# HugoZHL/MEVI

Measured on AMD Instinct MI355X. Metric: queries/sec @ MRR@10-match, MSMARCO dev, 1/2/4/8 MI355X, higher is better.
Workload: dtype f16+f32; 1 GPU; C2 dense arm (faiss_search.py Flat): 6980 x 768 f32 queries x 8841823 x 768 f32 docs, exact inner-product top-1000; queries=6980, docs=8841823, dim=768, topk=1000, parallelism=single GPU

## Files before the change

include/mevi_hip.h:

```cpp
#ifndef MEVI_HIP_H
#define MEVI_HIP_H

#include <stddef.h>
#include <stdint.h>

#ifdef __cplusplus
extern "C" {
#endif

#define MEVI_OK 0
#define MEVI_ERR_INVALID_ARG (-1)
#define MEVI_ERR_UNSUPPORTED (-2)
#define MEVI_ERR_WORKSPACE (-3)
#define MEVI_ERR_HIP (-4)

int mevi_abi_version(void);

const char *mevi_last_error(void);

size_t mevi_ip_topk_workspace_bytes(int64_t nq, int64_t dim, int64_t k);

int mevi_ip_topk_f32(const float *q, int64_t nq, const float *docs, int64_t nd,
                     int64_t dim, int64_t k, int64_t id_offset,
                     float *out_score, int64_t *out_id, void *workspace,
// ... 259 lines not shown
                            int64_t R, int pq, int32_t *labels, float *proba, void *workspace, size_t workspace_bytes,
                            void *stream);

size_t mevi_cluster_means_workspace_bytes(int64_t n, int64_t dim, int64_t K);
int mevi_cluster_means_f32(const float *x, int64_t n, int64_t dim, const int32_t *codes, int64_t code_stride,
                           int64_t K, const float *old_centroids, float *centroids, int32_t *counts, double *sum_sq,
                           void *workspace, size_t workspace_bytes, void *stream);

typedef struct mevi_ip_topk_stats {
  int64_t n_chunks;
  int64_t n_failed_queries;
  int64_t n_fallback_chunks;
  double filter_ms;
  double compact_ms;
  double filter_flops;
  double max_err_ratio;
  double err_bound;
  int64_t n_second_pass_queries;
  int64_t n_filter_candidates;
  int64_t max_launch_candidates;
  int64_t n_list_overflows;
  int64_t n_i8_queries;
  int64_t n_i8_unproven;
} mevi_ip_topk_stats;
int64_t mevi_ip_filter_tile_walk(int64_t n_dpairs, int64_t n_qtiles, int label, int32_t *dpair, int32_t *qtile);
void mevi_ip_topk_set_growth(double growth);
void mevi_ip_topk_set_profiling(int enable);
void mevi_ip_topk_get_stats(mevi_ip_topk_stats *out);

int64_t mevi_format_f32_list(const float *v, int64_t n, char *out, int64_t cap);
int64_t mevi_format_i64_list(const int64_t *v, int64_t n, char *out, int64_t cap);
int mevi_format_ranked_rows(const int64_t *ids, const float *scores, int64_t rows, int64_t k, char *out, int64_t row_cap,
                            int64_t *lens, int32_t threads);
int64_t mevi_parse_i64_list(const char *s, int64_t len, int64_t *out, int64_t cap);
int64_t mevi_parse_f64_list(const char *s, int64_t len, double *out, int64_t cap);

int64_t mevi_parse_tsv_columns(const char *buf, int64_t len, int32_t col_q, int32_t col_i, int32_t col_f, int64_t *q_span,
                               int64_t *seg_i, int64_t *vals_i, int64_t cap_i, int64_t *seg_f, double *vals_f,
                               int64_t cap_f, int64_t cap_lines);

int mevi_cluster_ranks_i32(const int32_t *codes, int64_t n_docs, int64_t M, const int64_t *docs, const int64_t *seg,
                           int64_t nq, const int32_t *beam, int64_t R, int32_t n_clusters, int32_t *out_ranks,
                           uint64_t *first_bad, void *stream);
int mevi_ensemble_rank_f64(const int64_t *seg_dense, const int64_t *docs_dense, const double *scores_dense,
                           const int32_t *cranks_dense, const int64_t *fine_row, const int64_t *seg_fine,
                           const int64_t *docs_fine, const double *scores_fine, int64_t nq, int64_t max_entries,
                           int32_t n_clusters, const double *term, double punish, const int64_t *out_seg,
                           int64_t *out_docs, int32_t *out_n, int32_t *err, void *stream);
// ... 8 lines not shown
```

mevi_amd/csrc/ip_topk.hip:

```cpp

#include "mfma_pp_f16x16.h"

#include <float.h>
#include <math.h>
#include <string.h>
#include <vector>

namespace mevi {
namespace {

constexpr int MAX_SORT = 16384;

struct TopkGeom {
  int k;
  int S;
  int cap;
};

static inline int next_pow2(int x) {
  int p = 1;
  while (p < x) p <<= 1;
  return p;
}

// ... 546 lines not shown
        base += __popcll(mask);
      }
    }
  for (int i = base + lane; i < k; i += 64) row[i] = (i == k - 1) ? T : 0ull;
  if (lane == 0) {
    tau[q] = (T != 0ull) ? key_score(T) : -INFINITY;
    count[q] = 0u;
    if (c_raw > (unsigned int)cap) failed[q] = 1u;
  }
}

template <int KPL>
__global__ __launch_bounds__(256) void rank_tau_kernel(const unsigned long long *__restrict__ buf, int nq, int S, int k, int rank,
                                                      float *__restrict__ tau, float *__restrict__ tau_s) {
  const int lane = threadIdx.x & 63;
  const int q = blockIdx.x * 4 + (int)(threadIdx.x >> 6);
  if (q >= nq) return;
  const unsigned long long *row = buf + (size_t)q * S;
  unsigned long long key[KPL];
#pragma unroll
  for (int j = 0; j < KPL; ++j) key[j] = (64 * j + lane < k) ? row[64 * j + lane] : 0ull;
  const int nj = (k + 63) >> 6;
  unsigned long long T = 0ull;
  for (int b = 63; b >= 0; --b) {
    const unsigned long long cand = T | (1ull << b);
    int cnt = 0;
#pragma unroll
    for (int jb = 0; jb < KPL / 8; ++jb)
      if (8 * jb < nj) {
#pragma unroll
        for (int jj = 0; jj < 8; ++jj) cnt += __popcll(__ballot(key[8 * jb + jj] >= cand));
      }
    if (cnt >= rank) T = cand;
  }
  if (lane == 0) {
    const float t = (T != 0ull) ? key_score(T) : -INFINITY;
    tau_s[q] = t;
    if (tau) tau[q] = t;
  }
}

__global__ __launch_bounds__(256) void sample_check_kernel(const float *__restrict__ tau, const float *__restrict__ tau_s,
                                                          unsigned int *__restrict__ failed, int nq) {
  const int q = blockIdx.x * 256 + threadIdx.x;
  if (q < nq && !(tau[q] > tau_s[q]) && tau_s[q] > -INFINITY) failed[q] = 1u;
}

__global__ __launch_bounds__(256) void sort_lists_kernel(unsigned long long *__restrict__ buf, int S, int k) {
  extern __shared__ __attribute__((aligned(16))) unsigned long long skeys[];
  const int t = threadIdx.x;
  unsigned long long *row = buf + (size_t)blockIdx.x * S;
  int P = 64;
  while (P < k) P <<= 1;
  for (int i = t; i < P; i += 256) skeys[i] = (i < k) ? row[i] : 0ull;
  __syncthreads();
  bitonic_sort_desc<256>(skeys, P, t);
// ... 942 lines not shown
    if (!ok) failed[q] = 1u;
  }
}

__global__ __launch_bounds__(256) void count_candidates_kernel(const unsigned int *__restrict__ count, int nq, int cap,
                                                              unsigned long long *__restrict__ out) {
  const int q = blockIdx.x * 256 + threadIdx.x;
  const unsigned int c = q < nq ? count[q] : 0u;
  unsigned long long sum = c;
  unsigned int mx = c, over = c > (unsigned int)cap ? 1u : 0u;
#pragma unroll
  for (int off = 32; off > 0; off >>= 1) {
    sum += ((unsigned long long)(unsigned int)__shfl_xor((int)(sum >> 32), off) << 32) | (unsigned int)__shfl_xor((int)sum, off);
    mx = max(mx, (unsigned int)__shfl_xor((int)mx, off));
    over += (unsigned int)__shfl_xor((int)over, off);
  }
  if ((threadIdx.x & 63) == 0 && sum != 0ull) {
    atomicAdd(out, sum);
    atomicMax(out + 1, (unsigned long long)mx);
    if (over) atomicAdd(out + 2, (unsigned long long)over);
  }
}

class Carver {
  char *base_;
  size_t used_ = 0;
 public:
  explicit Carver(void *base) : base_(static_cast<char *>(base)) {}
  template <typename T> T *take(size_t count) {
    T *p = base_ ? reinterpret_cast<T *>(base_ + used_) : nullptr;
    used_ += align_up(count * sizeof(T), 256);
    return p;
  }
  size_t used() const { return used_; }
};
template <typename F> static size_t carved_bytes(F &&carve) {
  Carver count(nullptr);
  carve(count);
  return count.used();
}

struct SearchState {
  unsigned long long *buf;
  unsigned int *count;
  float *tau;
  unsigned int *failed;
// ... 10 lines not shown
  SearchState st, fb;
  float *qsub; int *fidx;
  char *spare;
};
static ExactWs carve_exact(Carver &c, int64_t nq, int64_t dim, const TopkGeom &g) {
  return {carve_state(c, nq, g), carve_state(c, nq, g), c.take<float>((size_t)nq * dim), c.take<int>(nq), c.take<char>(256)};
}

struct QuerySide {
  float *image;
  float *norm, *inv, *delta, *n16;
  double *shift;
  unsigned int *err_bits;
};
static QuerySide carve_query_side(Carver &c, int64_t nq, size_t image_bytes) {
  QuerySide s = {reinterpret_cast<float *>(c.take<char>(image_bytes)), c.take<float>(nq + 1), c.take<float>(nq + 1),
                 c.take<float>(nq + 1), c.take<float>(nq + 1), c.take<double>(nq), nullptr};
  if (s.norm) s.err_bits = reinterpret_cast<unsigned int *>(s.norm + nq);
  return s;
}

thread_local double g_growth = 0.0;
thread_local int g_profile = 0;
thread_local mevi_ip_topk_stats g_stats = {0, 0, 0, 0.0, 0.0, 0.0, 0.0, 0.0, 0, 0, 0, 0};
thread_local std::vector<hipEvent_t> g_events;
thread_local std::vector<long long> g_chunk_rows;

static void profile_mark(hipStream_t stream) {
  if (!g_profile) return;
  hipEvent_t e;
  if (hipEventCreate(&e) != hipSuccess) return;
  (void)hipEventRecord(e, stream);
  g_events.push_back(e);
}

static void profile_collect() {
  for (size_t i = 0; i + 3 <= g_events.size(); i += 3) {
    float f = 0.f, c = 0.f;
    (void)hipEventElapsedTime(&f, g_events[i], g_events[i + 1]);
    (void)hipEventElapsedTime(&c, g_events[i + 1], g_events[i + 2]);
    g_stats.filter_ms += f;
    g_stats.compact_ms += c;
    if (getenv("MEVI_IP_TOPK_TRACE") && i / 3 < g_chunk_rows.size())
      fprintf(stderr, "ip_topk launch %zu: %lld rows  filter %.3f ms  compact %.3f ms\n", i / 3, g_chunk_rows[i / 3], f, c);
  }
  g_chunk_rows.clear();
  for (hipEvent_t e : g_events) (void)hipEventDestroy(e);
  g_events.clear();
}

enum class PassKind { ExactF32, F16Image, I8Image };
struct PassArgs {
  PassKind kind;
  const float *Q; int64_t nq;
  const float *D; int64_t nd; int dim;
  TopkGeom g; uint32_t id_base; SearchState st;
  bool guaranteed;
  unsigned long long *cand = nullptr;
  const float *row_scale = nullptr, *qub = nullptr;
};

enum class FilterGrid { PerTile, PerCU, SmallStream };
struct FilterChoice {
  const void *fn;
  size_t lds;
  int qt, ni16;
  FilterGrid grid;
};

static bool choose_filter(PassKind kind, int64_t nq, int dim, FilterChoice &f) {
  const bool h1 = kind != PassKind::ExactF32;
  const int ni = 2;
  static const bool shape32_f = [] { const char *e = getenv("MEVI_IP_FILTER_MFMA"); return e && atoi(e) == 32; }();
  static const int qt_pin = [] { const char *e = getenv("MEVI_IP_FILTER_QT"); return e ? atoi(e) : 0; }();
  const bool k16shape = h1 && !shape32_f && dim % 64 == 0;
  int ni16 = 8;
  if (k16shape) {
    ni16 = nq <= 64 ? 2 : (nq <= 128 ? 4 : 8);
    if (qt_pin == 256 || qt_pin == 128 || qt_pin == 64) ni16 = qt_pin / 32;
    const int nunits = dim / 32;
    if (ni16 == 2 && nunits < 5) ni16 = 4;
    if (ni16 == 4 && nunits < 4) ni16 = 8;
  }
// ... 25 lines not shown
}

static int64_t run_pass(const PassArgs &a, hipStream_t stream) {
  const int64_t nq = a.nq, nd = a.nd;
  const TopkGeom &g = a.g;
  const SearchState &st = a.st;
  const bool guaranteed = a.guaranteed;
  const long long total = nq * (long long)g.k;
  const long long init_n = total > nq ? total : nq;
  const int n_tickets = TICKET_SLOTS * 8;
  hipLaunchKernelGGL(init_state_kernel, dim3((unsigned)(((init_n > n_tickets ? init_n : n_tickets) + 255) / 256)), dim3(256), 0, stream,
                     st.buf, st.count, st.tau, st.failed, (long long)nq, g.S, g.k, st.tickets, n_tickets);
  const size_t compact_lds = (size_t)g.S * 8 + 2048;
  if (compact_lds > 65536) {
    if (hipFuncSetAttribute(reinterpret_cast<const void *>(compact_kernel),
                            hipFuncAttributeMaxDynamicSharedMemorySize, (int)compact_lds) != hipSuccess) {
      set_error("ip_topk: cannot raise dynamic LDS to %zu bytes", compact_lds);
      return -1;
    }
  }
  FilterChoice f;
  if (!choose_filter(a.kind, nq, a.dim, f)) return -1;
  const int n_qtiles = (int)((nq + f.qt - 1) / f.qt);
  double growth_div = 3.0;
  if (const char *e = getenv("MEVI_IP_TOPK_GROWTH_DIV")) {
    const double v = atof(e);
    if (v >= 1.05 && v <= 64.0) growth_div = v;
  }
  double growth = g_growth > 0.0 ? g_growth : (double)g.cap / (growth_div * g.k);
  if (growth < 1.0) growth = 1.0;
  if (g_growth <= 0.0 && !getenv("MEVI_IP_TOPK_GROWTH_DIV") && !guaranteed) {
    const double keys = (double)nq * (double)g.k * 60e-9 * 1e3, t_launch = 0.2;
    double best = growth, best_cost = (keys * growth + t_launch) / log(1.0 + growth);
    for (double cand = 1.0; cand < growth; cand += 0.25) {
      const double c = (keys * cand + t_launch) / log(1.0 + cand);
      if (c < best_cost * 0.99) best = cand, best_cost = c;
    }
    growth = best;
  }
  int64_t cap_docs = (g.cap / (2 * BM)) * (2 * BM);
  if (const char *e = getenv("MEVI_IP_TOPK_FIRST_CHUNK")) {
    const int64_t v = atoll(e) / (2 * BM) * (2 * BM);
    if (v >= 2 * BM && v < cap_docs) cap_docs = v;
  }
  if (hipFuncSetAttribute(f.fn, hipFuncAttributeMaxDynamicSharedMemorySize, (int)f.lds) != hipSuccess) {
    set_error("ip_topk: cannot raise dynamic LDS to %zu bytes", f.lds);
    return -1;
  }
  int n_cu = 256;
  {
    int dev = 0, v = 0;
    if (hipGetDevice(&dev) == hipSuccess &&
        hipDeviceGetAttribute(&v, hipDeviceAttributeMultiprocessorCount, dev) == hipSuccess && v >= 8)
      n_cu = v;
  }
  static const int cu_cap = [] { const char *e = getenv("MEVI_IP_FILTER_CUS"); return e ? atoi(e) : 0; }();
  if (cu_cap >= 8 && cu_cap < n_cu) n_cu = cu_cap / 8 * 8;
  static const int sample_mode = [] { const char *e = getenv("MEVI_IP_SAMPLE_TAU"); return e ? atoi(e) : -1; }();
  const bool sample_on = sample_mode == 1 || (sample_mode != 0 && nq <= 1024);
  double s_c = 0.0;
  int64_t n_sample = 0;
  bool sampled = false;
  if (sample_on && !guaranteed && g.k <= 4096 && g.k >= 32) {
    const double r = g.k / 2 < 16 ? 16.0 : (g.k / 2 > 96 ? 96.0 : (double)(g.k / 2));
    double c = r >= 96.0 ? 3.0 : 8.0;
    const double c_fit = (double)g.cap / ((double)g.k * (1.0 + 8.0 / sqrt(r)));
    if (c_fit < c) c = c_fit;
    if (c >= 1.5 && (1.0 - 1.0 / c) * sqrt(r) >= 4.5) {
      s_c = c;
      n_sample = (int64_t)ceil(r * (double)nd / (c * (double)g.k));
    }
  }
  int64_t seen = 0, launches = 0;
  while (seen < nd) {
    int64_t chunk = cap_docs;
    if (!guaranteed && seen >= g.k) {
      int64_t grown = (int64_t)((double)seen * growth);
      grown = grown / (2 * BM) * (2 * BM);
      if (grown > chunk) chunk = grown;
    }
    if (chunk > nd - seen) chunk = nd - seen;
    double expect_per_q = seen >= g.k ? (double)g.k * (double)chunk / (double)seen : (double)chunk;
    if (s_c > 0.0 && !sampled && seen >= n_sample && seen >= g.k && chunk < nd - seen) {
      const int64_t rank = (int64_t)ceil(s_c * (double)g.k * (double)seen / (double)nd);
      if (rank >= 16 && rank <= g.k) {
        hipLaunchKernelGGL(rank_tau_kernel<64>, dim3((unsigned)((nq + 3) / 4)), dim3(256), 0, stream, st.buf, (int)nq, g.S, g.k, (int)rank,
                           st.tau, st.tau_s);
        sampled = true;
        chunk = nd - seen;
        expect_per_q = s_c * (double)g.k;
      }
    }
    const int64_t n_dtiles = (chunk + 2 * BM - 1) / (2 * BM);
    const int64_t nwg = n_dtiles * n_qtiles;
    if (nwg > 0x7fffffffLL) {
      set_error("ip_topk: grid too large (%lld workgroups)", (long long)nwg);
      return -1;
    }
    profile_mark(stream);
    {
      int nq_i = (int)nq, n_dp = (int)n_dtiles, n_qt = n_qtiles;
      long long d0 = (long long)seen, d1 = (long long)(seen + chunk);
      const float *tau_c = st.tau;
      void *args[18] = {(void *)&a.Q, &nq_i, (void *)&a.D, &d0, &d1, (void *)&a.dim, (void *)&tau_c, (void *)&st.buf,
                        (void *)&st.count, (void *)&g.S, (void *)&g.k, (void *)&g.cap, (void *)&a.id_base};
      unsigned grid = (unsigned)nwg;
      int flush_mask = H16_FLUSH_EVERY - 1;
      unsigned int *tickets = st.tickets + 8 * (launches & 1), *tickets_next = st.tickets + 8 * ((launches + 1) & 1);
      if (f.grid == FilterGrid::SmallStream) {
        const int64_t nb = (chunk + 255) / 256;
        grid = (unsigned)(nb < n_cu ? nb : n_cu);
        args[13] = (void *)&a.row_scale;
        args[14] = (void *)&a.qub;
      } else {
// ... 2 lines not shown
          grid = (unsigned)(8 * per_xcd);
        }
        args[13] = &n_qt;
        args[14] = &n_dp;
      }
      if (f.ni16) {
        const double per_q = expect_per_q;
        const double r = per_q / (double)chunk * 64.0 * 16.0 * (double)f.ni16;
        int T = H16_FLUSH_EVERY;
        while (T > 1 && T * r > 56.0) T >>= 1;
        flush_mask = T - 1;
        args[15] = &flush_mask;
        args[16] = (void *)&tickets;
        args[17] = (void *)&tickets_next;
      }
      if (hipLaunchKernel(f.fn, dim3(grid), dim3(PP_THREADS), args, f.lds, stream) != hipSuccess) {
        set_error("ip_topk: filter kernel launch failed");
        return -1;
      }
    }
    profile_mark(stream);
    if (a.cand)
      hipLaunchKernelGGL(count_candidates_kernel, dim3((unsigned)((nq + 255) / 256)), dim3(256), 0, stream, st.count, (int)nq, g.cap, a.cand);
    {
      const int nq_i = (int)nq;
      static const bool wave_compact = [] { const char *e = getenv("MEVI_IP_TOPK_COMPACT"); return !(e && strcmp(e, "lds") == 0); }();
      if (wave_compact)
        hipLaunchKernelGGL(compact_wave_kernel<64>, dim3((unsigned)((nq + 3) / 4)), dim3(256), 0, stream, st.buf, st.count, st.tau,
                           st.failed, nq_i, g.S, g.k, g.cap);
      hipLaunchKernelGGL(compact_kernel, dim3((unsigned)(nq < 8 * n_cu ? nq : 8 * n_cu)), dim3(256), compact_lds, stream,
                         st.buf, st.count, st.tau, st.failed, nq_i, g.S, g.k, g.cap);
    }
    if (sampled && seen + chunk >= nd)
      hipLaunchKernelGGL(sample_check_kernel, dim3((unsigned)((nq + 255) / 256)), dim3(256), 0, stream, st.tau, st.tau_s, st.failed, (int)nq);
    profile_mark(stream);
    g_stats.filter_flops += 2.0 * (double)nq * (double)chunk * (double)a.dim;
    if (g_profile) g_chunk_rows.push_back((long long)chunk);
    seen += chunk;
    ++launches;
  }
  if (a.kind == PassKind::ExactF32)
    hipLaunchKernelGGL(sort_lists_kernel, dim3((unsigned)nq), dim3(256), (size_t)next_pow2(g.k < 64 ? 64 : g.k) * 8, stream,
                       st.buf, g.S, g.k);
  if (hipGetLastError() != hipSuccess) {
    set_error("ip_topk: kernel launch failed");
    return -1;
  }
  return launches;
}

static void finalize(const unsigned long long *lists, int ld, int64_t k, int64_t nq, float *out_score, int64_t *out_id, hipStream_t stream) {
  hipLaunchKernelGGL(finalize_kernel, dim3((unsigned)((nq * (long long)k + 255) / 256)), dim3(256), 0, stream, lists, ld, (int)k,
                     (long long)nq, out_score, reinterpret_cast<long long *>(out_id));
}

static void begin_call() {
  g_stats = {0, 0, 0, 0.0, 0.0, 0.0, 0.0, 0.0, 0, 0, 0, 0};
  for (hipEvent_t e : g_events) (void)hipEventDestroy(e);
  g_events.clear();
}

static int check_search(const char *who, bool index_needed, const float *q, int64_t nq, const float *docs, const void *index,
                        int64_t nd, int64_t dim, int64_t k, int64_t id_offset, const float *out_score, const int64_t *out_id,
                        const void *workspace, size_t workspace_bytes, size_t need) {
  MEVI_REQUIRE(nq >= 0 && nd >= 0 && dim > 0 && k > 0, MEVI_ERR_INVALID_ARG, "%s: bad shape nq=%lld nd=%lld dim=%lld k=%lld", who,
               (long long)nq, (long long)nd, (long long)dim, (long long)k);
  if (nq == 0) return MEVI_OK;
  MEVI_REQUIRE(q && out_score && out_id && (index || !index_needed) && (docs || nd == 0), MEVI_ERR_INVALID_ARG, "%s: null pointer", who);
  MEVI_REQUIRE(dim % 4 == 0 && k <= 4096, MEVI_ERR_UNSUPPORTED, "%s: dim %% 4 != 0 or k > 4096", who);
  MEVI_REQUIRE((uintptr_t)q % 16 == 0 && (uintptr_t)docs % 16 == 0 && (uintptr_t)index % 256 == 0, MEVI_ERR_INVALID_ARG,
               "%s: q/docs must be 16-byte, the index 256-byte aligned", who);
  MEVI_REQUIRE(id_offset >= 0 && id_offset + nd < 0xFFFFFFFFLL && nq < (1LL << 31) && (index_needed || dim < (1LL << 24)),
               MEVI_ERR_UNSUPPORTED, "%s: id_offset + nd, nq or dim out of range", who);
  MEVI_REQUIRE(workspace && workspace_bytes >= need, MEVI_ERR_WORKSPACE, "%s: workspace %zu bytes < required %zu", who, workspace_bytes, need);
  MEVI_REQUIRE((uintptr_t)workspace % 256 == 0, index_needed ? MEVI_ERR_WORKSPACE : MEVI_ERR_INVALID_ARG, "%s: misaligned workspace", who);
  return MEVI_OK;
}

static int exact_repair(const float *q, const std::vector<int> &idx, const float *docs, int64_t nd, int dim, const TopkGeom &g,
                        uint32_t id_base, const ExactWs &w, unsigned long long *dst, int dst_ld, bool restore_flops,
// ... 14 lines not shown
}

}
}

using namespace mevi;

extern "C" size_t mevi_ip_topk_workspace_bytes(int64_t nq, int64_t dim, int64_t k) {
  if (nq <= 0 || k <= 0 || k > 4096 || dim <= 0) return 0;
  return carved_bytes([&](Carver &c) { carve_exact(c, nq, dim, make_geom((int)k)); });
}

extern "C" int64_t mevi_ip_filter_tile_walk(int64_t n_dpairs, int64_t n_qtiles, int label, int32_t *dpair, int32_t *qtile) {
  if (n_dpairs <= 0 || n_qtiles <= 0 || n_dpairs * n_qtiles > 0x7fffffffLL || label < 0 || label > 7) return -1;
  int base, len;
  walk_range((int)(n_dpairs * n_qtiles), label, base, len);
  for (int t = 0; t < len && dpair && qtile; ++t) {
    int a, b;
    sweep_order(base + t, (int)n_dpairs, (int)n_qtiles, a, b);
    dpair[t] = a;
    qtile[t] = b;
  }
  return len;
}

extern "C" void mevi_ip_topk_set_growth(double growth) { g_growth = growth; }
extern "C" void mevi_ip_topk_set_profiling(int enable) { g_profile = enable; }

extern "C" void mevi_ip_topk_get_stats(mevi_ip_topk_stats *out) {
  if (out) *out = g_stats;
}

extern "C" int mevi_ip_topk_f32(const float *q, int64_t nq, const float *docs, int64_t nd, int64_t dim,
                                int64_t k, int64_t id_offset, float *out_score, int64_t *out_id,
                                void *workspace, size_t workspace_bytes, void *stream_) {
  hipStream_t stream = reinterpret_cast<hipStream_t>(stream_);
  begin_call();
  if (const int rc = check_search("ip_topk", false, q, nq, docs, nullptr, nd, dim, k, id_offset, out_score, out_id, workspace,
                                  workspace_bytes, mevi_ip_topk_workspace_bytes(nq, dim, k)))
    return rc;
  if (nq == 0) return MEVI_OK;

  const TopkGeom g = make_geom((int)k);
  Carver carver(workspace);
  const ExactWs w = carve_exact(carver, nq, dim, g);
  const SearchState &st = w.st;
// ... 137 lines not shown

extern "C" int mevi_ip_topk_indexed_f32(const float *q, int64_t nq, const float *docs, const void *index, int64_t nd,
                                        int64_t dim, int64_t k, int64_t id_offset, float *out_score,
                                        int64_t *out_id, void *workspace, size_t workspace_bytes, void *stream_) {
  hipStream_t stream = reinterpret_cast<hipStream_t>(stream_);
  begin_call();
  if (const int rc = check_search("ip_topk_indexed", true, q, nq, docs, index, nd, dim, k, id_offset, out_score, out_id, workspace,
                                  workspace_bytes, mevi_ip_topk_indexed_workspace_bytes(nq, dim, k)))
    return rc;
  if (nq == 0) return MEVI_OK;

  const int kp = h1_kprime((int)k);
  const TopkGeom gp = make_geom(kp, nq), g = make_geom((int)k);
  const int64_t dimp = pad_k(dim);
  IndexView iv = view_index(index, nd, dim);
  Carver carver(workspace);
  const IndexedWs w = carve_indexed(carver, nq, dim, k);
  const SearchState &st = w.first.st;
  const QuerySide &qs = w.first.qs;
  unsigned long long *const top = w.first.top;
  const float c1 = h1_cacc(dimp), c2 = h1_c2(dim);
  unsigned long long *cand = g_profile >= 2 ? w.counters : nullptr;
  if (cand) MEVI_HIP_CHECK(hipMemsetAsync(cand, 0, 32, stream));

  hipLaunchKernelGGL(split_queries_f16_kernel, dim3((unsigned)(image_rows(nq) / 4)), dim3(256), 0, stream, q, (long long)nq,
                     (int)dim, (int)dimp, iv.mu, iv.scal, reinterpret_cast<_Float16 *>(qs.image), qs.norm, qs.inv, qs.shift, qs.delta,
                     qs.n16);
  int64_t launches = run_pass({PassKind::F16Image, qs.image, nq, iv.image, nd, (int)dimp, gp, (uint32_t)id_offset, st, false, cand}, stream);
  if (launches < 0) return MEVI_ERR_HIP;
  g_stats.n_chunks = launches;
  g_stats.filter_flops *= (double)dim / (double)dimp;
  MEVI_HIP_CHECK(hipMemsetAsync(qs.err_bits, 0, 4, stream));
  {
    static const bool rescore_all = [] { const char *e = getenv("MEVI_IP_RESCORE_ALL"); return e && atoi(e) == 1; }();
    const float *acc_k = nullptr;
    if (!rescore_all && kp <= 4096 && k < kp) {
      hipLaunchKernelGGL(rank_tau_kernel<64>, dim3((unsigned)((nq + 3) / 4)), dim3(256), 0, stream, st.buf, (int)nq, gp.S, kp, (int)k,
                         (float *)nullptr, st.tau_s);
      acc_k = st.tau_s;
    }
    prove(q, docs, nq, dim, k, gp, (uint32_t)id_offset, st, qs, top, c1, c2, iv.bits, iv.norms_c, qs.err_bits, acc_k, 0, stream);
  }
  finalize(top, (int)k, k, nq, out_score, out_id, stream);
  float err_ratio = 0.f;
  MEVI_HIP_CHECK(hipMemcpyAsync(&err_ratio, qs.err_bits, 4, hipMemcpyDeviceToHost, stream));
  unsigned long long cand_host[3] = {0ull, 0ull, 0ull};
  if (cand) MEVI_HIP_CHECK(hipMemcpyAsync(cand_host, cand, 24, hipMemcpyDeviceToHost, stream));
  MEVI_HIP_CHECK(hipGetLastError());
  std::vector<unsigned int> failed((size_t)nq);
  MEVI_HIP_CHECK(hipMemcpyAsync(failed.data(), st.failed, (size_t)nq * 4, hipMemcpyDeviceToHost, stream));
  MEVI_HIP_CHECK(hipStreamSynchronize(stream));
// ... 1 lines not shown
  g_stats.max_err_ratio = err_ratio;
  g_stats.err_bound = 1.0;
  g_stats.n_filter_candidates = (int64_t)cand_host[0];
  g_stats.max_launch_candidates = (int64_t)cand_host[1];
  g_stats.n_list_overflows = (int64_t)cand_host[2];
  const bool bound_suspect = g_stats.max_err_ratio > 1.0;
  std::vector<int> idx;
  for (int64_t i = 0; i < nq; ++i)
    if (failed[(size_t)i] || bound_suspect) idx.push_back((int)i);
  const bool repaired = !idx.empty();
  const int kp2 = h1_kprime2((int)k);
  if (!idx.empty() && !bound_suspect && kp2 != 0 && (int64_t)idx.size() <= h1_second_pass_max(nq)) {
    const int64_t n2 = (int64_t)idx.size();
    g_stats.n_second_pass_queries = n2;
    const TopkGeom g2 = make_geom(kp2);
    const SearchState &s2 = w.second.st;
    const QuerySide &qs2 = w.second.qs;
    MEVI_HIP_CHECK(hipMemcpyAsync(w.idx2, idx.data(), (size_t)n2 * 4, hipMemcpyHostToDevice, stream));
    hipLaunchKernelGGL(gather_rows_kernel, dim3((unsigned)n2), dim3(256), 0, stream, q, w.idx2, (int)n2, (int)dim, w.q2);
    hipLaunchKernelGGL(split_queries_f16_kernel, dim3((unsigned)(image_rows(n2) / 4)), dim3(256), 0, stream, w.q2, (long long)n2,
                       (int)dim, (int)dimp, iv.mu, iv.scal, reinterpret_cast<_Float16 *>(qs2.image), qs2.norm, qs2.inv, qs2.shift,
                       qs2.delta, qs2.n16);
    const double keep_flops = g_stats.filter_flops;
    const int64_t l2 = run_pass({PassKind::F16Image, qs2.image, n2, iv.image, nd, (int)dimp, g2, (uint32_t)id_offset, s2, false}, stream);
    g_stats.filter_flops = keep_flops;
    if (l2 < 0) return MEVI_ERR_HIP;
    prove(w.q2, docs, n2, dim, k, g2, (uint32_t)id_offset, s2, qs2, w.second.top, c1, c2, iv.bits, iv.norms_c, nullptr, nullptr, 0,
          stream);
    hipLaunchKernelGGL(scatter_top_kernel, dim3((unsigned)n2), dim3(256), 0, stream, w.second.top, w.idx2, (int)n2, (int)k, (int)k, top,
                       (int)k);
    std::vector<unsigned int> failed2((size_t)n2);
    MEVI_HIP_CHECK(hipMemcpyAsync(failed2.data(), s2.failed, (size_t)n2 * 4, hipMemcpyDeviceToHost, stream));
    MEVI_HIP_CHECK(hipStreamSynchronize(stream));
    profile_collect();
    std::vector<int> still;
    for (int64_t i = 0; i < n2; ++i)
      if (failed2[(size_t)i]) still.push_back(idx[(size_t)i]);
    idx.swap(still);
  }
  if (!idx.empty())
    if (const int rc = exact_repair(q, idx, docs, nd, (int)dim, g, (uint32_t)id_offset, w.exact, top, (int)k, true, stream)) return rc;
  if (repaired) finalize(top, (int)k, k, nq, out_score, out_id, stream);
  MEVI_HIP_CHECK(hipGetLastError());
  return MEVI_OK;
}

namespace {
struct Index8View {
// ... 204 lines not shown
```

mevi_amd/hip.py:

```python
import ctypes
import os
from ctypes import c_double, c_float, c_int, c_int64, c_size_t, c_void_p

import torch

from .build import LIB

_lib = None


class MeviHipError(RuntimeError):
    pass


class IpTopkStats(ctypes.Structure):
    _fields_ = [("n_chunks", c_int64), ("n_failed_queries", c_int64), ("n_fallback_chunks", c_int64),
                ("filter_ms", c_double), ("compact_ms", c_double), ("filter_flops", c_double),
                ("max_err_ratio", c_double), ("err_bound", c_double), ("n_second_pass_queries", c_int64),
                ("n_filter_candidates", c_int64), ("max_launch_candidates", c_int64), ("n_list_overflows", c_int64),
                ("n_i8_queries", c_int64), ("n_i8_unproven", c_int64)]


_SIGNATURES = {
    "mevi_abi_version": (c_int, []),
    "mevi_last_error": (ctypes.c_char_p, []),
    "mevi_ip_topk_workspace_bytes": (c_size_t, [c_int64, c_int64, c_int64]),
    "mevi_ip_topk_f32": (c_int, [c_void_p, c_int64, c_void_p, c_int64, c_int64, c_int64, c_int64,
                                 c_void_p, c_void_p, c_void_p, c_size_t, c_void_p]),
    "mevi_ip_index_bytes": (c_size_t, [c_int64, c_int64]),
    "mevi_ip_index_build_f32": (c_int, [c_void_p, c_int64, c_int64, c_void_p, c_size_t, c_void_p]),
    "mevi_ip_topk_indexed_workspace_bytes": (c_size_t, [c_int64, c_int64, c_int64]),
    "mevi_ip_topk_indexed_f32": (c_int, [c_void_p, c_int64, c_void_p, c_void_p, c_int64, c_int64, c_int64, c_int64,
                                         c_void_p, c_void_p, c_void_p, c_size_t, c_void_p]),
    "mevi_ip_index8_bytes": (c_size_t, [c_int64, c_int64]),
    "mevi_ip_index8_build_f32": (c_int, [c_void_p, c_void_p, c_int64, c_int64, c_void_p, c_size_t, c_void_p]),
    "mevi_ip_topk_indexed8_workspace_bytes": (c_size_t, [c_int64, c_int64, c_int64]),
    "mevi_ip_topk_indexed8_f32": (c_int, [c_void_p, c_int64, c_void_p, c_void_p, c_void_p, c_int64, c_int64, c_int64, c_int64,
                                          c_void_p, c_void_p, c_void_p, c_size_t, c_void_p]),
    "mevi_topk_merge_workspace_bytes": (c_size_t, [c_int64, c_int64, c_int64, c_int64]),
    "mevi_topk_merge_f32": (c_int, [c_void_p, c_void_p, c_int64, c_int64, c_int64, c_int64,
                                    c_void_p, c_void_p, c_void_p, c_size_t, c_void_p]),
    "mevi_pack_lists_i64": (c_int, [c_void_p, c_void_p, c_int64, c_void_p, c_void_p]),
    "mevi_topk_merge_packed_f32": (c_int, [c_void_p, c_int64, c_int64, c_int64, c_int64, c_int, c_void_p, c_void_p, c_void_p,
# ... 111 lines not shown
    "mevi_rq_beam_encode_workspace_bytes": (c_size_t, [c_int64, c_int64, c_int64, c_int64, c_int64, c_int]),
    "mevi_rq_beam_encode_tile_docs": (c_int64, [c_int64, c_int64, c_int64, c_int64, c_int]),
    "mevi_rq_beam_encode_f32": (c_int, [c_void_p, c_int64, c_int64, c_void_p, c_int64, c_int64, c_int64, c_int, c_void_p,
                                        c_void_p, c_void_p, c_size_t, c_void_p]),
    "mevi_cluster_means_workspace_bytes": (ctypes.c_size_t, [c_int64, c_int64, c_int64]),
    "mevi_cluster_means_f32": (c_int, [c_void_p, c_int64, c_int64, c_void_p, c_int64, c_int64, c_void_p, c_void_p, c_void_p,
                               c_void_p, c_void_p, ctypes.c_size_t, c_void_p]),
    "mevi_format_f32_list": (c_int64, [c_void_p, c_int64, c_void_p, c_int64]),
    "mevi_format_i64_list": (c_int64, [c_void_p, c_int64, c_void_p, c_int64]),
    "mevi_format_ranked_rows": (c_int, [c_void_p, c_void_p, c_int64, c_int64, c_void_p, c_int64, c_void_p, ctypes.c_int32]),
    "mevi_parse_i64_list": (c_int64, [ctypes.c_char_p, c_int64, c_void_p, c_int64]),
    "mevi_parse_f64_list": (c_int64, [ctypes.c_char_p, c_int64, c_void_p, c_int64]),
    "mevi_parse_tsv_columns": (c_int64, [c_void_p, c_int64, ctypes.c_int32, ctypes.c_int32, ctypes.c_int32, c_void_p,
                                         c_void_p, c_void_p, c_int64, c_void_p, c_void_p, c_int64, c_int64]),
    "mevi_cluster_ranks_i32": (c_int, [c_void_p, c_int64, c_int64, c_void_p, c_void_p, c_int64, c_void_p, c_int64,
                                       ctypes.c_int32, c_void_p, c_void_p, c_void_p]),
    "mevi_ensemble_rank_f64": (c_int, [c_void_p, c_void_p, c_void_p, c_void_p, c_void_p, c_void_p, c_void_p, c_void_p, c_int64,
                                       c_int64, ctypes.c_int32, c_void_p, c_double, c_void_p, c_void_p, c_void_p, c_void_p,
                                       c_void_p]),
    "mevi_first_hits_i64": (c_int, [c_void_p, c_void_p, c_void_p, c_void_p, c_void_p, c_int64, c_void_p, c_void_p]),
    "mevi_ip_filter_tile_walk": (c_int64, [c_int64, c_int64, c_int, c_void_p, c_void_p]),
    "mevi_ip_topk_set_growth": (None, [c_double]),
    "mevi_ip_topk_set_profiling": (None, [c_int]),
    "mevi_ip_topk_get_stats": (None, [ctypes.POINTER(IpTopkStats)]),
}


_FINE_AGG_SIGNATURES = {
    "mevi_fine_topk_agg_workspace_bytes": (c_size_t, [c_int64, c_int64, c_int64, c_int64, c_int64, c_int]),
    "mevi_fine_topk_agg_query_tile": (c_int64, [c_int64, c_int64, c_int64, c_int64, c_int64, c_int]),
    "mevi_fine_topk_agg_f32": (c_int, [c_void_p, c_int64, c_int, c_int64, c_int64, c_void_p, c_int64, c_int64, c_void_p, c_void_p,
                                       c_void_p, c_int64, c_void_p, c_int64, c_int64, c_int, c_void_p, c_void_p, c_float, c_float,
                                       c_void_p, c_void_p, c_void_p, c_void_p, c_void_p, c_size_t, c_void_p]),
}


_ATTN_LONG_SIGNATURES = {
    "mevi_attention_long_f32": _SIGNATURES["mevi_attention_f32"],
    "mevi_attention_long_varlen_f32": _SIGNATURES["mevi_attention_varlen_f32"],
    "mevi_attention_long_route": (c_int, _SIGNATURES["mevi_attention_f32"][1][:-1]),
    "mevi_attention_long_varlen_route": (c_int, _SIGNATURES["mevi_attention_varlen_f32"][1][:-1]),
}
ATTN_LONG_MAX_KEYS = 2048
ATTN_LONG_ROUTES = {"LONG_MFMA": 13, "LONG_ROWS": 14}


# ... 92 lines not shown
```

Measured before the change: 83460 queries/s.

## Plan filter launches ahead with speculative rank thresholds from measured count dispersion

Moves the chunk-growth schedule into a launch planner. After one early chunk it measures the variance-to-mean ratio of per-query candidate counts with a host sync, then re-plans the remaining documents into fewer, larger launches. Each of those launches uses a speculative rank-based threshold (rank_tau_kernel) checked afterwards by sample_check. The z-budget is sized so failed queries stay rare, and failures fall back to the existing second pass. The rank search also exits early on an exact count match. This trades fewer compact passes and launches for a mid-pass sync and some risk of failed queries or cap overflow.

```diff
diff --git a/include/mevi_hip.h b/include/mevi_hip.h
--- a/include/mevi_hip.h
+++ b/include/mevi_hip.h
@@ -305,8 +305,12 @@
   int64_t n_list_overflows;
   int64_t n_i8_queries;
   int64_t n_i8_unproven;
+  int64_t n_predicted_launches;
+  double dispersion;
 } mevi_ip_topk_stats;
 int64_t mevi_ip_filter_tile_walk(int64_t n_dpairs, int64_t n_qtiles, int label, int32_t *dpair, int32_t *qtile);
+int64_t mevi_ip_topk_plan(int64_t nq, int64_t nd, int64_t kprime, int64_t cap, double dispersion, int64_t max_launches,
+                          int64_t *rows, int32_t *rank, double *expect_keys);
 void mevi_ip_topk_set_growth(double growth);
 void mevi_ip_topk_set_profiling(int enable);
 void mevi_ip_topk_get_stats(mevi_ip_topk_stats *out);
diff --git a/mevi_amd/csrc/ip_topk.hip b/mevi_amd/csrc/ip_topk.hip
--- a/mevi_amd/csrc/ip_topk.hip
+++ b/mevi_amd/csrc/ip_topk.hip
@@ -592,6 +592,7 @@
   for (int j = 0; j < KPL; ++j) key[j] = (64 * j + lane < k) ? row[64 * j + lane] : 0ull;
   const int nj = (k + 63) >> 6;
   unsigned long long T = 0ull;
+  bool exact = false;
   for (int b = 63; b >= 0; --b) {
     const unsigned long long cand = T | (1ull << b);
     int cnt = 0;
@@ -601,7 +602,32 @@
 #pragma unroll
         for (int jj = 0; jj < 8; ++jj) cnt += __popcll(__ballot(key[8 * jb + jj] >= cand));
       }
-    if (cnt >= rank) T = cand;
+    if (cnt >= rank) {
+      T = cand;
+      if (cnt == rank) {
+        exact = true;
+        break;
+      }
+    }
+  }
+  if (exact) {
+    unsigned long long mn = ~0ull;
+#pragma unroll
+    for (int jb = 0; jb < KPL / 8; ++jb)
+      if (8 * jb < nj) {
+#pragma unroll
+        for (int jj = 0; jj < 8; ++jj) {
+          const unsigned long long kk = key[8 * jb + jj];
+          if (kk >= T && kk < mn) mn = kk;
+        }
+      }
+#pragma unroll
+    for (int off = 32; off > 0; off >>= 1) {
+      const unsigned long long o = ((unsigned long long)(unsigned int)__shfl_xor((int)(mn >> 32), off) << 32) |
+                                   (unsigned int)__shfl_xor((int)mn, off);
+      mn = o < mn ? o : mn;
+    }
+    T = mn;
   }
   if (lane == 0) {
     const float t = (T != 0ull) ? key_score(T) : -INFINITY;
@@ -1590,6 +1616,22 @@
   }
 }
 
+__global__ __launch_bounds__(256) void count_moments_kernel(const unsigned int *__restrict__ count, int nq,
+                                                           unsigned long long *__restrict__ out) {
+  const int q = blockIdx.x * 256 + threadIdx.x;
+  const unsigned long long c = q < nq ? count[q] : 0u;
+  unsigned long long s1 = c, s2 = c * c;
+#pragma unroll
+  for (int off = 32; off > 0; off >>= 1) {
+    s1 += ((unsigned long long)(unsigned int)__shfl_xor((int)(s1 >> 32), off) << 32) | (unsigned int)__shfl_xor((int)s1, off);
+    s2 += ((unsigned long long)(unsigned int)__shfl_xor((int)(s2 >> 32), off) << 32) | (unsigned int)__shfl_xor((int)s2, off);
+  }
+  if ((threadIdx.x & 63) == 0 && s1 != 0ull) {
+    atomicAdd(out, s1);
+    atomicAdd(out + 1, s2);
+  }
+}
+
 class Carver {
   char *base_;
   size_t used_ = 0;
@@ -1646,7 +1688,7 @@
 
 thread_local double g_growth = 0.0;
 thread_local int g_profile = 0;
-thread_local mevi_ip_topk_stats g_stats = {0, 0, 0, 0.0, 0.0, 0.0, 0.0, 0.0, 0, 0, 0, 0};
+thread_local mevi_ip_topk_stats g_stats = {0, 0, 0, 0.0, 0.0, 0.0, 0.0, 0.0, 0, 0, 0, 0, 0, 0, 0, 0.0};
 thread_local std::vector<hipEvent_t> g_events;
 thread_local std::vector<long long> g_chunk_rows;
 
@@ -1682,7 +1724,151 @@
   bool guaranteed;
   unsigned long long *cand = nullptr;
   const float *row_scale = nullptr, *qub = nullptr;
+  unsigned long long *moments = nullptr;
 };
+
+struct PlanLaunch {
+  int64_t rows;
+  int rank;
+  double expect;
+};
+struct PlanShape {
+  int64_t nq, nd;
+  int k, cap;
+  bool guaranteed;
+  bool predict;
+  double D;
+};
+
+static bool spec_tau_on() {
+  static const bool on = [] { const char *e = getenv("MEVI_IP_SPEC_TAU"); return !(e && atoi(e) == 0); }();
+  return on;
+}
+static int64_t spec_min_seen() {
+  static const int64_t v = [] { const char *e = getenv("MEVI_IP_SPEC_MIN_SEEN"); const long long x = e ? atoll(e) : 0; return x >= 1000 ? (int64_t)x : (int64_t)50000; }();
+  return v;
+}
+constexpr double SPEC_D_NONE = 64.0;
+constexpr double T_KEY_MS = 30e-9, T_LAUNCH_MS = 0.44;
+
+static double spec_z(int64_t nq, int launches) {
+  const double budget = 1e-3 / ((double)nq * (double)launches);
+  double lo = 0.0, hi = 12.0;
+  for (int i = 0; i < 60; ++i) {
+    const double mid = 0.5 * (lo + hi);
+    (0.5 * erfc(mid / sqrt(2.0)) <= budget ? hi : lo) = mid;
+  }
+  return hi;
+}
+
+static bool spec_launch(int64_t seen, int64_t chunk, int k, int cap, double D, double z, PlanLaunch &out) {
+  const double frac = (double)seen / (double)(seen + chunk);
+  for (double c = 1.15; c * (double)k <= (double)cap; c += 0.01) {
+    const double r = ceil(c * (double)k * frac);
+    if (r < 16.0 || r > (double)k) continue;
+    if ((1.0 - 1.0 / c) * sqrt(r / D) < z) continue;
+    if (c * (double)k * (1.0 + z * sqrt(D / r)) > (double)cap) return false;
+    const double appended = c * (double)k * (1.0 - frac);
+    if (2 * k <= 64 * 64 && (double)k + appended * (1.0 + 2.0 * sqrt(D / r)) > 64.0 * 64.0) return false;
+    out = {chunk, (int)r, appended};
+    return true;
+  }
+  return false;
+}
+
+static std::vector<PlanLaunch> plan_pass(const PlanShape &p) {
+  const int64_t nq = p.nq, nd = p.nd;
+  const int k = p.k, cap = p.cap;
+  const bool guaranteed = p.guaranteed;
+  double growth_div = 3.0;
+  if (const char *e = getenv("MEVI_IP_TOPK_GROWTH_DIV")) {
+    const double v = atof(e);
+    if (v >= 1.05 && v <= 64.0) growth_div = v;
+  }
+  double growth = g_growth > 0.0 ? g_growth : (double)cap / (growth_div * k);
+  if (growth < 1.0) growth = 1.0;
+  if (g_growth <= 0.0 && !getenv("MEVI_IP_TOPK_GROWTH_DIV") && !guaranteed) {
+    const double keys = (double)nq * (double)k * 60e-9 * 1e3, t_launch = 0.2;
+    double best = growth, best_cost = (keys * growth + t_launch) / log(1.0 + growth);
+    for (double cand = 1.0; cand < growth; cand += 0.25) {
+      const double c = (keys * cand + t_launch) / log(1.0 + cand);
+      if (c < best_cost * 0.99) best = cand, best_cost = c;
+    }
+    growth = best;
+  }
+  int64_t cap_docs = (cap / (2 * BM)) * (2 * BM);
+  if (const char *e = getenv("MEVI_IP_TOPK_FIRST_CHUNK")) {
+    const int64_t v = atoll(e) / (2 * BM) * (2 * BM);
+    if (v >= 2 * BM && v < cap_docs) cap_docs = v;
+  }
+  static const int sample_mode = [] { const char *e = getenv("MEVI_IP_SAMPLE_TAU"); return e ? atoi(e) : -1; }();
+  const bool sample_on = sample_mode == 1 || (sample_mode != 0 && nq <= 1024);
+  double s_c = 0.0;
+  int64_t n_sample = 0;
+  bool sampled = false;
+  if (sample_on && !guaranteed && k <= 4096 && k >= 32) {
+    const double r = k / 2 < 16 ? 16.0 : (k / 2 > 96 ? 96.0 : (double)(k / 2));
+    double c = r >= 96.0 ? 3.0 : 8.0;
+    const double c_fit = (double)cap / ((double)k * (1.0 + 8.0 / sqrt(r)));
+    if (c_fit < c) c = c_fit;
+    if (c >= 1.5 && (1.0 - 1.0 / c) * sqrt(r) >= 4.5) {
+      s_c = c;
+      n_sample = (int64_t)ceil(r * (double)nd / (c * (double)k));
+    }
+  }
+  const bool predict = p.predict && !sample_on && !guaranteed && nq > 1024 && k >= 32 && k <= 4096 && p.D < SPEC_D_NONE && p.D >= 1.0;
+  int spec_left = -1;
+  double spec_zv = 0.0;
+  std::vector<PlanLaunch> plan;
+  int64_t seen = 0;
+  while (seen < nd) {
+    int64_t chunk = cap_docs;
+    if (!guaranteed && seen >= k) {
+      int64_t grown = (int64_t)((double)seen * growth);
+      grown = grown / (2 * BM) * (2 * BM);
+      if (grown > chunk) chunk = grown;
+    }
+    if (chunk > nd - seen) chunk = nd - seen;
+    PlanLaunch l = {chunk, 0, seen >= k ? (double)k * (double)chunk / (double)seen : (double)chunk};
+    if (s_c > 0.0 && !sampled && seen >= n_sample && seen >= k && chunk < nd - seen) {
+      const int64_t rank = (int64_t)ceil(s_c * (double)k * (double)seen / (double)nd);
+      if (rank >= 16 && rank <= k) {
+        sampled = true;
+        l = {nd - seen, (int)rank, s_c * (double)k};
+      }
+    }
+    if (predict && seen >= spec_min_seen() && seen >= k && chunk < nd - seen) {
+      const double ratio = (double)nd / (double)seen;
+      const auto step = [&](int n_left) {
+        if (n_left <= 1) return nd - seen;
+        const int64_t c = (int64_t)((double)seen * (pow(ratio, 1.0 / n_left) - 1.0)) / (2 * BM) * (2 * BM);
+        return c < nd - seen ? c : nd - seen;
+      };
+      if (spec_left < 0) {
+        spec_left = 0;
+        const int n_exact = (int)ceil(log(ratio) / log(1.0 + (double)chunk / (double)seen));
+        double best_cost = (double)n_exact * ((double)nq * l.expect * T_KEY_MS + T_LAUNCH_MS);
+        for (int n = 1; n < n_exact; ++n) {
+          const double z = spec_z(nq, n);
+          PlanLaunch t;
+          const int64_t c = step(n);
+          if (c < 2 * BM || !spec_launch(seen, c, k, cap, p.D, z, t)) continue;
+          const double cost = (double)n * ((double)nq * t.expect * T_KEY_MS + T_LAUNCH_MS);
+          if (cost < best_cost) best_cost = cost, spec_left = n, spec_zv = z;
+        }
+      }
+      if (spec_left > 0) {
+        PlanLaunch t;
+        const int64_t c = step(spec_left);
+        if (c >= 2 * BM && spec_launch(seen, c, k, cap, p.D, spec_zv, t)) l = t;
+        if (l.rows == c) --spec_left;
+      }
+    }
+    plan.push_back(l);
+    seen += l.rows;
+  }
+  return plan;
+}
 
 enum class FilterGrid { PerTile, PerCU, SmallStream };
 struct FilterChoice {
@@ -1754,27 +1940,6 @@
   FilterChoice f;
   if (!choose_filter(a.kind, nq, a.dim, f)) return -1;
   const int n_qtiles = (int)((nq + f.qt - 1) / f.qt);
-  double growth_div = 3.0;
-  if (const char *e = getenv("MEVI_IP_TOPK_GROWTH_DIV")) {
-    const double v = atof(e);
-    if (v >= 1.05 && v <= 64.0) growth_div = v;
-  }
-  double growth = g_growth > 0.0 ? g_growth : (double)g.cap / (growth_div * g.k);
-  if (growth < 1.0) growth = 1.0;
-  if (g_growth <= 0.0 && !getenv("MEVI_IP_TOPK_GROWTH_DIV") && !guaranteed) {
-    const double keys = (double)nq * (double)g.k * 60e-9 * 1e3, t_launch = 0.2;
-    double best = growth, best_cost = (keys * growth + t_launch) / log(1.0 + growth);
-    for (double cand = 1.0; cand < growth; cand += 0.25) {
-      const double c = (keys * cand + t_launch) / log(1.0 + cand);
-      if (c < best_cost * 0.99) best = cand, best_cost = c;
-    }
-    growth = best;
-  }
-  int64_t cap_docs = (g.cap / (2 * BM)) * (2 * BM);
-  if (const char *e = getenv("MEVI_IP_TOPK_FIRST_CHUNK")) {
-    const int64_t v = atoll(e) / (2 * BM) * (2 * BM);
-    if (v >= 2 * BM && v < cap_docs) cap_docs = v;
-  }
   if (hipFuncSetAttribute(f.fn, hipFuncAttributeMaxDynamicSharedMemorySize, (int)f.lds) != hipSuccess) {
     set_error("ip_topk: cannot raise dynamic LDS to %zu bytes", f.lds);
     return -1;
@@ -1788,40 +1953,43 @@
   }
   static const int cu_cap = [] { const char *e = getenv("MEVI_IP_FILTER_CUS"); return e ? atoi(e) : 0; }();
   if (cu_cap >= 8 && cu_cap < n_cu) n_cu = cu_cap / 8 * 8;
-  static const int sample_mode = [] { const char *e = getenv("MEVI_IP_SAMPLE_TAU"); return e ? atoi(e) : -1; }();
-  const bool sample_on = sample_mode == 1 || (sample_mode != 0 && nq <= 1024);
-  double s_c = 0.0;
-  int64_t n_sample = 0;
-  bool sampled = false;
-  if (sample_on && !guaranteed && g.k <= 4096 && g.k >= 32) {
-    const double r = g.k / 2 < 16 ? 16.0 : (g.k / 2 > 96 ? 96.0 : (double)(g.k / 2));
-    double c = r >= 96.0 ? 3.0 : 8.0;
-    const double c_fit = (double)g.cap / ((double)g.k * (1.0 + 8.0 / sqrt(r)));
-    if (c_fit < c) c = c_fit;
-    if (c >= 1.5 && (1.0 - 1.0 / c) * sqrt(r) >= 4.5) {
-      s_c = c;
-      n_sample = (int64_t)ceil(r * (double)nd / (c * (double)g.k));
-    }
-  }
+  PlanShape shape = {nq, nd, g.k, g.cap, guaranteed, a.kind == PassKind::F16Image && a.moments && spec_tau_on(), 1e30};
+  static const double d_pin = [] { const char *e = getenv("MEVI_IP_SPEC_D"); return e ? atof(e) : 0.0; }();
+  if (shape.predict && d_pin >= 1.0) shape.D = d_pin;
+  std::vector<PlanLaunch> plan = plan_pass(shape);
+  int64_t measure_at = -1;
+  if (shape.predict && !(d_pin >= 1.0)) {
+    int64_t s = 0;
+    for (size_t i = 0; i + 1 < plan.size(); s += plan[i++].rows)
+      if (s + plan[i].rows >= spec_min_seen()) {
+        if (s >= g.k && plan[i].rank == 0) measure_at = (int64_t)i;
+        break;
+      }
+  }
+  if (shape.predict) g_stats.dispersion = d_pin >= 1.0 ? d_pin : 0.0;
+  static const bool trace = getenv("MEVI_IP_TOPK_TRACE") != nullptr;
+  const auto trace_plan = [&](const char *what) {
+    if (!trace) return;
+    int64_t s = 0;
+    for (size_t i = 0; i < plan.size(); s += plan[i++].rows)
+      fprintf(stderr, "ip_topk plan (%s, D = %.3g) launch %zu: rows %lld -> %lld  rank %d  expected keys %.0f\n", what,
+              shape.predict ? shape.D : 0.0, i, (long long)s, (long long)(s + plan[i].rows), plan[i].rank, plan[i].expect);
+  };
+  trace_plan(shape.predict && measure_at >= 0 ? "before D" : "final");
   int64_t seen = 0, launches = 0;
   while (seen < nd) {
-    int64_t chunk = cap_docs;
-    if (!guaranteed && seen >= g.k) {
-      int64_t grown = (int64_t)((double)seen * growth);
-      grown = grown / (2 * BM) * (2 * BM);
-      if (grown > chunk) chunk = grown;
-    }
-    if (chunk > nd - seen) chunk = nd - seen;
-    double expect_per_q = seen >= g.k ? (double)g.k * (double)chunk / (double)seen : (double)chunk;
-    if (s_c > 0.0 && !sampled && seen >= n_sample && seen >= g.k && chunk < nd - seen) {
-      const int64_t rank = (int64_t)ceil(s_c * (double)g.k * (double)seen / (double)nd);
-      if (rank >= 16 && rank <= g.k) {
-        hipLaunchKernelGGL(rank_tau_kernel<64>, dim3((unsigned)((nq + 3) / 4)), dim3(256), 0, stream, st.buf, (int)nq, g.S, g.k, (int)rank,
-                           st.tau, st.tau_s);
-        sampled = true;
-        chunk = nd - seen;
-        expect_per_q = s_c * (double)g.k;
-      }
+    if ((size_t)launches >= plan.size()) {
+      set_error("ip_topk: the launch plan ends at row %lld of %lld", (long long)seen, (long long)nd);
+      return -1;
+    }
+    const PlanLaunch pl = plan[(size_t)launches];
+    const int64_t chunk = pl.rows;
+    const double expect_per_q = pl.expect;
+    const bool predicted = pl.rank > 0;
+    if (predicted) {
+      hipLaunchKernelGGL(rank_tau_kernel<64>, dim3((unsigned)((nq + 3) / 4)), dim3(256), 0, stream, st.buf, (int)nq, g.S, g.k, pl.rank,
+                         st.tau, st.tau_s);
+      ++g_stats.n_predicted_launches;
     }
     const int64_t n_dtiles = (chunk + 2 * BM - 1) / (2 * BM);
     const int64_t nwg = n_dtiles * n_qtiles;
@@ -1870,6 +2038,8 @@
     profile_mark(stream);
     if (a.cand)
       hipLaunchKernelGGL(count_candidates_kernel, dim3((unsigned)((nq + 255) / 256)), dim3(256), 0, stream, st.count, (int)nq, g.cap, a.cand);
+    if (launches == measure_at)
+      hipLaunchKernelGGL(count_moments_kernel, dim3((unsigned)((nq + 255) / 256)), dim3(256), 0, stream, st.count, (int)nq, a.moments);
     {
       const int nq_i = (int)nq;
       static const bool wave_compact = [] { const char *e = getenv("MEVI_IP_TOPK_COMPACT"); return !(e && strcmp(e, "lds") == 0); }();
@@ -1879,13 +2049,33 @@
       hipLaunchKernelGGL(compact_kernel, dim3((unsigned)(nq < 8 * n_cu ? nq : 8 * n_cu)), dim3(256), compact_lds, stream,
                          st.buf, st.count, st.tau, st.failed, nq_i, g.S, g.k, g.cap);
     }
-    if (sampled && seen + chunk >= nd)
+    if (predicted)
       hipLaunchKernelGGL(sample_check_kernel, dim3((unsigned)((nq + 255) / 256)), dim3(256), 0, stream, st.tau, st.tau_s, st.failed, (int)nq);
     profile_mark(stream);
     g_stats.filter_flops += 2.0 * (double)nq * (double)chunk * (double)a.dim;
     if (g_profile) g_chunk_rows.push_back((long long)chunk);
     seen += chunk;
     ++launches;
+    if (launches - 1 == measure_at) {
+      unsigned long long m[2] = {0ull, 0ull};
+      if (hipMemcpyAsync(m, a.moments, sizeof(m), hipMemcpyDeviceToHost, stream) != hipSuccess ||
+          hipStreamSynchronize(stream) != hipSuccess) {
+        set_error("ip_topk: reading the dispersion sums failed");
+        return -1;
+      }
+      const double mean = (double)m[0] / (double)nq, var = (double)m[1] / (double)nq - mean * mean;
+      const double ratio = mean >= 1.0 ? var / mean / (1.0 + (double)chunk / (double)(seen - chunk)) : 1e30;
+      shape.D = ratio > 1.0 ? ratio : 1.0;
+      g_stats.dispersion = shape.D;
+      plan = plan_pass(shape);
+      trace_plan("final");
+      int64_t s = 0;
+      for (size_t i = 0; i < (size_t)launches && i < plan.size(); ++i) s += plan[i].rows;
+      if (s != seen) {
+        set_error("ip_topk: the launch plan changed behind row %lld", (long long)seen);
+        return -1;
+      }
+    }
   }
   if (a.kind == PassKind::ExactF32)
     hipLaunchKernelGGL(sort_lists_kernel, dim3((unsigned)nq), dim3(256), (size_t)next_pow2(g.k < 64 ? 64 : g.k) * 8, stream,
@@ -1903,7 +2093,7 @@
 }
 
 static void begin_call() {
-  g_stats = {0, 0, 0, 0.0, 0.0, 0.0, 0.0, 0.0, 0, 0, 0, 0};
+  g_stats = {0, 0, 0, 0.0, 0.0, 0.0, 0.0, 0.0, 0, 0, 0, 0, 0, 0, 0, 0.0};
   for (hipEvent_t e : g_events) (void)hipEventDestroy(e);
   g_events.clear();
 }
@@ -1964,6 +2154,19 @@
     qtile[t] = b;
   }
   return len;
+}
+
+extern "C" int64_t mevi_ip_topk_plan(int64_t nq, int64_t nd, int64_t kprime, int64_t cap, double dispersion, int64_t max_launches,
+                                     int64_t *rows, int32_t *rank, double *expect_keys) {
+  if (nq <= 0 || nd < 0 || kprime <= 0 || kprime > MAX_SORT || cap < 2 * BM || cap > MAX_SORT || !(dispersion >= 1.0) || max_launches < 0)
+    return -1;
+  const std::vector<PlanLaunch> plan = plan_pass({nq, nd, (int)kprime, (int)cap, false, spec_tau_on(), dispersion});
+  for (size_t i = 0; i < plan.size() && (int64_t)i < max_launches; ++i) {
+    if (rows) rows[i] = plan[i].rows;
+    if (rank) rank[i] = plan[i].rank;
+    if (expect_keys) expect_keys[i] = plan[i].expect;
+  }
+  return (int64_t)plan.size();
 }
 
 extern "C" void mevi_ip_topk_set_growth(double growth) { g_growth = growth; }
@@ -2147,11 +2350,14 @@
   const float c1 = h1_cacc(dimp), c2 = h1_c2(dim);
   unsigned long long *cand = g_profile >= 2 ? w.counters : nullptr;
   if (cand) MEVI_HIP_CHECK(hipMemsetAsync(cand, 0, 32, stream));
+  unsigned long long *const moments = w.counters + 4;
+  MEVI_HIP_CHECK(hipMemsetAsync(moments, 0, 16, stream));
 
   hipLaunchKernelGGL(split_queries_f16_kernel, dim3((unsigned)(image_rows(nq) / 4)), dim3(256), 0, stream, q, (long long)nq,
                      (int)dim, (int)dimp, iv.mu, iv.scal, reinterpret_cast<_Float16 *>(qs.image), qs.norm, qs.inv, qs.shift, qs.delta,
                      qs.n16);
-  int64_t launches = run_pass({PassKind::F16Image, qs.image, nq, iv.image, nd, (int)dimp, gp, (uint32_t)id_offset, st, false, cand}, stream);
+  int64_t launches = run_pass({PassKind::F16Image, qs.image, nq, iv.image, nd, (int)dimp, gp, (uint32_t)id_offset, st, false, cand,
+                               nullptr, nullptr, moments}, stream);
   if (launches < 0) return MEVI_ERR_HIP;
   g_stats.n_chunks = launches;
   g_stats.filter_flops *= (double)dim / (double)dimp;
@@ -2199,8 +2405,10 @@
                        (int)dim, (int)dimp, iv.mu, iv.scal, reinterpret_cast<_Float16 *>(qs2.image), qs2.norm, qs2.inv, qs2.shift,
                        qs2.delta, qs2.n16);
     const double keep_flops = g_stats.filter_flops;
+    const int64_t keep_predicted = g_stats.n_predicted_launches;
     const int64_t l2 = run_pass({PassKind::F16Image, qs2.image, n2, iv.image, nd, (int)dimp, g2, (uint32_t)id_offset, s2, false}, stream);
     g_stats.filter_flops = keep_flops;
+    g_stats.n_predicted_launches = keep_predicted;
     if (l2 < 0) return MEVI_ERR_HIP;
     prove(w.q2, docs, n2, dim, k, g2, (uint32_t)id_offset, s2, qs2, w.second.top, c1, c2, iv.bits, iv.norms_c, nullptr, nullptr, 0,
           stream);
diff --git a/mevi_amd/hip.py b/mevi_amd/hip.py
--- a/mevi_amd/hip.py
+++ b/mevi_amd/hip.py
@@ -18,7 +18,8 @@
                 ("filter_ms", c_double), ("compact_ms", c_double), ("filter_flops", c_double),
                 ("max_err_ratio", c_double), ("err_bound", c_double), ("n_second_pass_queries", c_int64),
                 ("n_filter_candidates", c_int64), ("max_launch_candidates", c_int64), ("n_list_overflows", c_int64),
-                ("n_i8_queries", c_int64), ("n_i8_unproven", c_int64)]
+                ("n_i8_queries", c_int64), ("n_i8_unproven", c_int64),
+                ("n_predicted_launches", c_int64), ("dispersion", c_double)]
 
 
 _SIGNATURES = {
@@ -176,6 +177,7 @@
     "mevi_ip_filter_tile_walk": (c_int64, [c_int64, c_int64, c_int, c_void_p, c_void_p]),
     "mevi_ip_topk_set_growth": (None, [c_double]),
     "mevi_ip_topk_set_profiling": (None, [c_int]),
+    "mevi_ip_topk_plan": (c_int64, [c_int64, c_int64, c_int64, c_int64, c_double, c_int64, c_void_p, c_void_p, c_void_p]),
     "mevi_ip_topk_get_stats": (None, [ctypes.POINTER(IpTopkStats)]),
 }
 
```

Measured after the change: 85230 queries/s (median of 6 runs). 1.02x the previous value.
